# guy3540/Acoustic_Locating_VQ-VAE

Hardware: AMD Instinct MI355X
Metric: spectrograms/sec (train step), speech VQ-VAE default config (higher is better)
Workload: dtype x3mx_hb

## Files before the change

acoustic_locating_vq-vae_amd/csrc/wgrad_reduce.h:

```cpp
#pragma once
#include "alvq_common.h"

namespace alvq {

static __device__ __forceinline__ void wgrad_reduce_body(const float* partial, float* dw, int splits, int KW, int M, int C,
                                                         int w_layout, int accumulate, const float* scale, long stride, int bid,
                                                         int nblk) {
  const long total = (long)KW * M * C;
  const float sc = scale ? *scale : 1.f;
  if (w_layout == ALVQ_W_OIK && KW == 3) {
    const long pairs = (long)M * C;
    for (long q = bid * 256L + threadIdx.x; q < pairs; q += (long)nblk * 256) {
      float s0 = 0.f, s1 = 0.f, s2 = 0.f;
      const float* p = partial + q;
      int k = 0;
      for (; k + 2 <= splits; k += 2) {
        const float* pa = p + (long)k * stride;
        const float* pb = pa + stride;
        const float a0 = pa[0], a1 = pa[pairs], a2 = pa[2 * pairs], b0 = pb[0], b1 = pb[pairs], b2 = pb[2 * pairs];
        s0 = (s0 + a0) + b0;
        s1 = (s1 + a1) + b1;
        s2 = (s2 + a2) + b2;
      }
      for (; k < splits; ++k) {
        const float* pa = p + (long)k * stride;
        s0 += pa[0];
        s1 += pa[pairs];
        s2 += pa[2 * pairs];
      }
      if (scale) { s0 *= sc; s1 *= sc; s2 *= sc; }
      float* o = dw + 3 * q;
      if (accumulate) { s0 += o[0]; s1 += o[1]; s2 += o[2]; }
      o[0] = s0; o[1] = s1; o[2] = s2;
    }
    return;
  }
  for (long e = bid * 256L + threadIdx.x; e < total; e += (long)nblk * 256) {
    int m, c, t;
    if (w_layout == ALVQ_W_OIK) {
      t = (int)(e % KW);
      c = (int)((e / KW) % C);
      m = (int)(e / ((long)KW * C));
    } else {
      const int tt = (int)(e % KW);
      t = KW - 1 - tt;
      m = (int)((e / KW) % M);
      c = (int)(e / ((long)KW * M));
    }
    const long src = ((long)t * M + m) * C + c;
    float s = 0.f;
    int k = 0;
    for (; k + 4 <= splits; k += 4) {
      const float v0 = partial[(long)k * stride + src], v1 = partial[(long)(k + 1) * stride + src],
                  v2 = partial[(long)(k + 2) * stride + src], v3 = partial[(long)(k + 3) * stride + src];
      s = (((s + v0) + v1) + v2) + v3;
    }
    for (; k < splits; ++k) s += partial[(long)k * stride + src];
    if (scale) s *= sc;
    dw[e] = accumulate ? dw[e] + s : s;
  }
}
static __global__ void wgrad_reduce_kernel(const float* partial, float* dw, int splits, int KW, int M, int C, int w_layout,
                                    int accumulate, const float* scale) {
  wgrad_reduce_body(partial, dw, splits, KW, M, C, w_layout, accumulate, scale, (long)KW * M * C, blockIdx.x, gridDim.x);
}

template <int RB>
static __device__ __forceinline__ void wgrad_reduce_iok_body(float (&tile)[3][RB][65], const float* partial, float* dw, int splits,
                                                             int KW, int M, int C, int accumulate, const float* scale, int bid) {
  constexpr int RI = RB / 8;
  const int ctiles = (C + 63) / 64;
  const int m0 = (bid / ctiles) * RB, c0 = (bid % ctiles) * 64;
  const int tx = threadIdx.x & 31, ty = threadIdx.x >> 5;
  const long plane = (long)M * C, total = (long)KW * plane;
  const bool pair = (C % 2 == 0);
  float s0[3][RI], s1[3][RI];
#pragma unroll
  for (int t = 0; t < 3; ++t)
#pragma unroll
    for (int i = 0; i < RI; ++i) s0[t][i] = s1[t][i] = 0.f;
  const int c = c0 + 2 * tx;
  const bool full = pair && m0 + RB <= M && c0 + 64 <= C;
  if (full) {
    const float* p0 = partial + (long)(m0 + ty) * C + c;
    if (KW == 3) {
#pragma unroll 4
      for (int k = 0; k < splits; ++k) {
        float2 v[3][RI];
#pragma unroll
        for (int t = 0; t < 3; ++t)
#pragma unroll
          for (int i = 0; i < RI; ++i) v[t][i] = *(const float2*)(p0 + (long)k * total + (long)t * plane + (long)(8 * i) * C);
#pragma unroll
        for (int t = 0; t < 3; ++t)
#pragma unroll
          for (int i = 0; i < RI; ++i) {
            s0[t][i] += v[t][i].x;
            s1[t][i] += v[t][i].y;
          }
      }
    } else {
#pragma unroll 4
      for (int k = 0; k < splits; ++k) {
        float2 v[RI];
#pragma unroll
        for (int i = 0; i < RI; ++i) v[i] = *(const float2*)(p0 + (long)k * total + (long)(8 * i) * C);
#pragma unroll
        for (int i = 0; i < RI; ++i) {
          s0[0][i] += v[i].x;
          s1[0][i] += v[i].y;
        }
      }
    }
  } else
  for (int k = 0; k < splits; ++k) {
    const float* pk = partial + (long)k * total + c;
#pragma unroll
    for (int t = 0; t < 3; ++t) {
      if (t >= KW) break;
#pragma unroll
      for (int i = 0; i < RI; ++i) {
        const int m = m0 + ty + 8 * i;
        if (m >= M) continue;
        const float* p = pk + (long)t * plane + (long)m * C;
        if (pair && c + 1 < C) {
          const float2 v = *(const float2*)p;
          s0[t][i] += v.x;
          s1[t][i] += v.y;
        } else {
          if (c < C) s0[t][i] += p[0];
          if (c + 1 < C) s1[t][i] += p[1];
        }
      }
    }
  }
#pragma unroll
  for (int t = 0; t < 3; ++t) {
    if (t >= KW) break;
#pragma unroll
    for (int i = 0; i < RI; ++i) {
      tile[t][ty + 8 * i][2 * tx] = s0[t][i];
      tile[t][ty + 8 * i][2 * tx + 1] = s1[t][i];
    }
  }
  __syncthreads();
  const int run = RB * KW;
  for (int e = threadIdx.x; e < 64 * run; e += 256) {
    const int cc = e / run, j = e - cc * run, mr = j / KW, tt = j - mr * KW;
    if (c0 + cc >= C || m0 + mr >= M) continue;
    const long o = ((long)(c0 + cc) * M + m0) * KW + j;
    float v = tile[KW - 1 - tt][mr][cc];
    if (scale) v *= *scale;
    dw[o] = accumulate ? dw[o] + v : v;
  }
}
template <int RB>
static __global__ __launch_bounds__(256) void wgrad_reduce_iok_kernel(const float* partial, float* dw, int splits, int KW,
                                                                      int M, int C, int accumulate, const float* scale) {
  __shared__ float tile[3][RB][65];
  wgrad_reduce_iok_body<RB>(tile, partial, dw, splits, KW, M, C, accumulate, scale, blockIdx.x);
}

static inline void wgrad_reduce_launch(const float* partial, float* dw, int splits, int KW, int M, int C, int w_layout,
                                       int accumulate, hipStream_t s, const float* scale = nullptr) {
  if (w_layout == ALVQ_W_IOK) {
    const int grid = ((M + 15) / 16) * ((C + 63) / 64);
    hipLaunchKernelGGL(wgrad_reduce_iok_kernel<16>, dim3(grid), dim3(256), 0, s, partial, dw, splits, KW, M, C, accumulate, scale);
    return;
  }
  const long total = (long)KW * M * C;
  int rgrid = (int)((total + 255) / 256);
  if (rgrid > 2048) rgrid = 2048;
  hipLaunchKernelGGL(wgrad_reduce_kernel, dim3(rgrid), dim3(256), 0, s, partial, dw, splits, KW, M, C, w_layout, accumulate, scale);
}

}
```

acoustic_locating_vq-vae_amd/csrc/wgrad_reduce_batch.hip:

```cpp
#include "alvq_common.h"
#include "wgrad_reduce.h"

namespace alvq {

constexpr int RB_MAX = 40;
struct ReduceBatch {
  alvq_reduce_desc d[RB_MAX];
  int blk0[RB_MAX];
  int nblk[RB_MAX];
  int n;
};

__global__ __launch_bounds__(256) void wgrad_reduce_batch_kernel(ReduceBatch b) {
  __shared__ float tile[3][16][65];
  int di = 0;
  for (int i = 1; i < b.n; ++i)
    if ((int)blockIdx.x >= b.blk0[i]) di = i;
  const alvq_reduce_desc& d = b.d[di];
  const int lb = blockIdx.x - b.blk0[di];
  const int acc = d.accumulate;
  if (d.w_layout == ALVQ_W_IOK && d.stride == (int64_t)d.KW * d.M * d.C)
    wgrad_reduce_iok_body<16>(tile, d.partial, d.dst, d.splits, d.KW, d.M, d.C, acc, d.scale, lb);
  else
    wgrad_reduce_body(d.partial, d.dst, d.splits, d.KW, d.M, d.C, d.w_layout, acc, d.scale, (long)d.stride, lb, b.nblk[di]);
}

}

using namespace alvq;

extern "C" int alvq_wgrad_reduce_batch(const alvq_reduce_desc* descs, int n, void* stream) {
  ALVQ_REQUIRE(descs && n > 0, ALVQ_EINVAL, "alvq_wgrad_reduce_batch: no descriptors");
  for (int i = 0; i < n; ++i) {
    const alvq_reduce_desc& s = descs[i];
    ALVQ_REQUIRE(s.partial && s.dst, ALVQ_EINVAL, "alvq_wgrad_reduce_batch: null pointer in descriptor %d", i);
    ALVQ_REQUIRE(s.splits >= 1 && s.splits <= 64 && s.M > 0 && s.C > 0 && (s.KW == 1 || s.KW == 3), ALVQ_EINVAL,
                 "alvq_wgrad_reduce_batch: bad dims in descriptor %d", i);
    ALVQ_REQUIRE(s.w_layout == ALVQ_W_OIK || s.w_layout == ALVQ_W_IOK, ALVQ_EINVAL, "alvq_wgrad_reduce_batch: w_layout in descriptor %d", i);
    ALVQ_REQUIRE(s.stride >= (int64_t)s.KW * s.M * s.C, ALVQ_EINVAL, "alvq_wgrad_reduce_batch: stride in descriptor %d", i);
  }
  for (int i0 = 0; i0 < n; i0 += RB_MAX) {
    ReduceBatch b{};
    b.n = n - i0 < RB_MAX ? n - i0 : RB_MAX;
    int blocks = 0;
    for (int i = 0; i < b.n; ++i) {
      const alvq_reduce_desc& s = descs[i0 + i];
      b.d[i] = s;
      const long total = (long)s.KW * s.M * s.C;
      int nb;
      if (s.w_layout == ALVQ_W_IOK && s.stride == total) nb = ((s.M + 15) / 16) * ((s.C + 63) / 64);
      else {
        nb = (int)((total + 255) / 256);
        if (nb > 2048) nb = 2048;
      }
      b.blk0[i] = blocks;
      b.nblk[i] = nb;
      blocks += nb;
    }
    hipLaunchKernelGGL(wgrad_reduce_batch_kernel, dim3(blocks), dim3(256), 0, (hipStream_t)stream, b);
    int rc = check_launch("alvq_wgrad_reduce_batch");
    if (rc) return rc;
  }
  return ALVQ_OK;
}
```

acoustic_locating_vq-vae_amd/src/acoustic_locating_vq_vae/_native.py:

```python
from __future__ import annotations

import collections
import ctypes
import functools
import os

import torch

_LIB = None
_HERE = os.path.dirname(os.path.abspath(__file__))
_DEFAULT_LIB = os.path.normpath(os.path.join(_HERE, "..", "..", "lib", "libalvq.so"))

W_OIK = 0
W_IOK = 1
VQ_PARTIALS = 1024
EW_PARTIALS = 1024

_c_void_p = ctypes.c_void_p
_i32 = ctypes.c_int
_i64 = ctypes.c_int64
_f32 = ctypes.c_float

_SIGNATURES = {
    "alvq_version": (ctypes.c_char_p, []),
# ... 258 lines not shown
        rc = lib().alvq_conv1d_f32(_ptr(x, name="x"), _ptr(w, name="w"), _ptr(bias, name="bias"), _ptr(skip1, name="skip1"),
                                   _ptr(skip2, name="skip2"), _ptr(mask, name="mask"), _ptr(post, name="post"),
                                   _ptr(y), _ptr(y2), B, C, M, L, KW, w_layout, int(bool(relu)), _stream())
    _check(rc, "alvq_conv1d_f32")
    return (y, y2) if post is not None else y


_WS = {}
_WS_RETIRED = []


def _workspace(nbytes, device):
    key = (device.type, device.index, torch.cuda.current_stream(device).cuda_stream)
    buf = _WS.get(key)
    if buf is None or buf.numel() < nbytes:
        if buf is not None:
            _WS_RETIRED.append(buf)
        buf = torch.empty(max(nbytes, 1 << 20), device=device, dtype=torch.uint8)
        _WS[key] = buf
    return buf


WGRAD_DEFER = 2
_ARENA = {}


class ReduceDesc(ctypes.Structure):
    _fields_ = [("partial", ctypes.c_void_p), ("dst", ctypes.c_void_p), ("scale", ctypes.c_void_p), ("splits", ctypes.c_int32),
                ("KW", ctypes.c_int32), ("M", ctypes.c_int32), ("C", ctypes.c_int32), ("w_layout", ctypes.c_int32),
                ("accumulate", ctypes.c_int32), ("stride", ctypes.c_int64)]


def arena_reset(device):
    key = (device.type, device.index, torch.cuda.current_stream(device).cuda_stream)
    st = _ARENA.get(key)
    if st is not None:
        st["chunk"], st["off"] = 0, 0


def arena_alloc(nbytes, device):
    key = (device.type, device.index, torch.cuda.current_stream(device).cuda_stream)
    st = _ARENA.setdefault(key, {"chunks": [], "chunk": 0, "off": 0})
    nbytes = (nbytes + 255) // 256 * 256
    while True:
        if st["chunk"] >= len(st["chunks"]):
            st["chunks"].append(torch.empty(max(nbytes, 256 << 20), device=device, dtype=torch.uint8))
            st["off"] = 0
        buf = st["chunks"][st["chunk"]]
        if st["off"] + nbytes <= buf.numel():
            ptr = buf.data_ptr() + st["off"]
            st["off"] += nbytes
            return ptr
        st["chunk"] += 1
        st["off"] = 0


class DeferredReductions(list):

    def __init__(self):
        super().__init__()
        self.keep = []


def wgrad_reduce_batch(descs):
    if not descs:
        return
    arr = (ReduceDesc * len(descs))(*descs)
    _check(lib().alvq_wgrad_reduce_batch(ctypes.addressof(arr), len(descs), _stream()), "alvq_wgrad_reduce_batch")
    if isinstance(descs, DeferredReductions):
        descs.keep.clear()


def _defer_descs(defer, ws_ptr, dw, dbias, scale, nseg, B, C, M, L, KW, w_layout):
    L_ = lib()
    scale_ptr = _sptr(scale, 1)
    dsts = {dw.data_ptr()} | ({dbias.data_ptr()} if dbias is not None else set())
    if any(d.dst in dsts for d in defer):
        wgrad_reduce_batch(defer)
        del defer[:]
    if scale is not None and hasattr(defer, "keep"):
        defer.keep.append(scale)
    splits = L_.alvq_conv1d_wgrad_bf16_splits(B, C, M, L, KW, nseg, int(dbias is not None))
    defer.append(ReduceDesc(ws_ptr, dw.data_ptr(), scale_ptr, splits, KW, M, C, w_layout, 1, KW * M * C))
    if dbias is not None:
        off = L_.alvq_conv1d_wgrad_bf16_bias_offset(B, C, M, L, KW)
        defer.append(ReduceDesc(ws_ptr + off, dbias.data_ptr(), scale_ptr, splits, 1, 1, M, W_OIK, 1, (M + 63) // 64 * 64))


def conv1d_wgrad(dy, x, KW, w_layout=W_OIK, want_bias=False, dw_out=None, dbias_out=None, accumulate=False):
# ... 1054 lines not shown
```

acoustic_locating_vq-vae_amd/src/acoustic_locating_vq_vae/_ops.py:

```python
from __future__ import annotations

import os

import numpy as np
import torch

from . import _native as N

OIK, IOK = N.W_OIK, N.W_IOK

DEFAULT_DTYPE = "x3mx_hb"
MODES = ("x3mx_hb", "f16mx_hb", "bf16x3_hb", "f32", "bf16")
INTERNAL_MODES = ("f16mx", "bf16x3", "f16mx_hd")
_DTYPE = os.environ.get("ALVQ_DTYPE", DEFAULT_DTYPE)
if _DTYPE not in MODES:
    raise ValueError("ALVQ_DTYPE must be one of %s, got %r" % (", ".join(repr(m) for m in MODES), _DTYPE))


def set_compute_dtype(name, internal=False):
    global _DTYPE
    if name not in MODES and not (internal and name in INTERNAL_MODES):
        raise ValueError("compute dtype must be one of %s, got %r" % (", ".join(repr(m) for m in MODES), name))
    _DTYPE = name

# ... 15 lines not shown
    for p in params:
        if p.grad is not None:
            _GRAD_SINKS[p.data_ptr()] = p.grad


_SINKS_ACTIVE = 0


class use_grad_sinks:

    def __enter__(self):
        global _SINKS_ACTIVE
        _SINKS_ACTIVE += 1

    def __exit__(self, *exc):
        global _SINKS_ACTIVE
        _SINKS_ACTIVE -= 1


_DEFERRED = None


class deferred_reduce:
    def __enter__(self):
        global _DEFERRED
        self.prev, _DEFERRED = _DEFERRED, (N.DeferredReductions() if os.environ.get("ALVQ_DEFER_REDUCE", "1") != "0" else None)
        return _DEFERRED

    def __exit__(self, *exc):
        global _DEFERRED
        _DEFERRED = self.prev


_API_FORWARDS = 0


def note_training_forward(device):
    global _API_FORWARDS
    if device.type != "cuda" or _SINKS_ACTIVE or not has_fp16_range() or torch.cuda.is_current_stream_capturing():
        return
    every = int(os.environ.get("ALVQ_RANGE_CHECK_EVERY", "200"))
    _API_FORWARDS += 1
    if every <= 0 or _API_FORWARDS < every:
        return
    _API_FORWARDS = 0
    flag = N.f16mx_range_flag(reset=True, device=device)
    if flag:
        import warnings
        warnings.warn("acoustic_locating_vq_vae: fp16 range flag %d in mode %s -- a value entering or produced inside the "
# ... 136 lines not shown
    def __exit__(self, *exc):
        global _LATENT_TAP
        _LATENT_TAP = self.prev



class use_pack_pool:

    def __init__(self, pool, refresh=True):
        self.pool, self.do_refresh = pool, refresh

    def __enter__(self):
        global _ACTIVE_POOL
        self.prev, _ACTIVE_POOL = _ACTIVE_POOL, self.pool
        if self.pool is not None and self.do_refresh:
            self.pool.refresh()

    def __exit__(self, *exc):
        global _ACTIVE_POOL
        _ACTIVE_POOL = self.prev


def _defer_kw(eng, sink):
    return {"defer": _DEFERRED} if (_DEFERRED is not None and sink is not None and eng.can_defer) else {}


def _wgrad(eng, dy, x, kw, layout, w, b=None, dw_prev=None):
    if b is not None and not b.requires_grad:
        b = None
    if not w.requires_grad:
        if b is None:
            return None, None
        raise RuntimeError("a convolution with a frozen weight and a trainable bias is not supported on the HIP path")
    sw, sb = _sink(w), _sink(b)
    if sw is not None and (b is None or sb is not None):
        eng.wgrad(dy, x, kw, layout, want_bias=b is not None, dw_out=sw, dbias_out=sb, accumulate=True, **_defer_kw(eng, sw))
        return None, None
    if b is not None:
        dw, db = eng.wgrad(dy, x, kw, layout, want_bias=True, dw_out=dw_prev, accumulate=dw_prev is not None)
        return dw, db
    return eng.wgrad(dy, x, kw, layout, dw_out=dw_prev, accumulate=dw_prev is not None), None


def dense(x):
    if isinstance(x, StandardisedT):
        return x.materialise()
    if x.dtype != torch.float32:
# ... 560 lines not shown
```

acoustic_locating_vq-vae_amd/src/acoustic_locating_vq_vae/train_step.py:

```python
from __future__ import annotations

import os

import torch
import torch.distributed as dist

from . import _native as N
from . import _ops

_ALIGN = 64


def _round_up(n):
    return (n + _ALIGN - 1) // _ALIGN * _ALIGN


def _world_rank(group=None, without=(1, 0)):
    if not (dist.is_available() and dist.is_initialized()):
        return without
    return dist.get_world_size(group), dist.get_rank(group)


def unique_trainable(params):
    seen, out = set(), []
# ... 9 lines not shown
    def __init__(self, params, extra=0):
        self.params = unique_trainable(params)
        if not self.params:
            raise ValueError("no trainable parameters")
        dev = self.params[0].device
        self.offsets, total = [], _ALIGN
        for p in self.params:
            if p.device != dev or p.dtype != torch.float32:
                raise ValueError("all parameters must be fp32 on one device")
            self.offsets.append(total)
            total += _round_up(p.numel())
        self.extra_span = (total, total + extra) if extra else None
        total += _round_up(extra)
        self.numel = sum(p.numel() for p in self.params)
        self.flat = torch.zeros(total, device=dev, dtype=torch.float32)
        self.grad = torch.zeros(total, device=dev, dtype=torch.float32)
        for p, off in zip(self.params, self.offsets):
            n = p.numel()
            self.flat[off:off + n].copy_(p.data.reshape(-1))
            p.data = self.flat[off:off + n].view(p.shape)
            p.grad = self.grad[off:off + n].view(p.shape)
        self.skip_slot = self.grad[0:1]

    def zero_grad(self):
        if self.grad.is_cuda:
            N.fill_(self.grad, 0.0)
        else:
            self.grad.zero_()
        for p, off in zip(self.params, self.offsets):
            if p.grad is None or p.grad.data_ptr() != self.grad.data_ptr() + 4 * off:
                p.grad = self.grad[off:off + p.numel()].view(p.shape)

    def sync_grads(self, group=None, force=False):
        world = _world_rank(group, without=(0, 0))[0]
        if world == 0 or (world == 1 and not force):
            return 1.0
        dist.all_reduce(self.grad, op=dist.ReduceOp.SUM, group=group)
        return 1.0 / world

    def span(self, params):
        ids = {id(p) for p in params}
        idx = [i for i, p in enumerate(self.params) if id(p) in ids]
        if not idx or idx != list(range(idx[0], idx[-1] + 1)) or len(idx) != len(ids):
            raise ValueError("bucket parameters are not a contiguous run of the flat buffer")
        last = idx[-1]
        hi = self.offsets[last + 1] if last + 1 < len(self.offsets) else self.grad.numel()
        return (0 if idx[0] == 0 else self.offsets[idx[0]]), hi

    def sync_span(self, lo, hi, group=None, force=False):
        world = _world_rank(group, without=(0, 0))[0]
        if world == 0 or (world == 1 and not force):
            return None
        return dist.all_reduce(self.grad[lo:hi], op=dist.ReduceOp.SUM, group=group, async_op=True)

    def broadcast_params(self, src=0, group=None):
        if _world_rank(group)[0] > 1:
            dist.broadcast(self.flat, src=src, group=group)


class WarmupCosine:

    __slots__ = ("warmup_steps", "total_steps", "lr_min")

    def __init__(self, warmup_steps, total_steps=None, lr_min=0.0):
        if int(warmup_steps) != warmup_steps or warmup_steps < 0:
            raise ValueError("WarmupCosine: warmup_steps=%r must be an integer >= 0" % (warmup_steps,))
        if total_steps is not None and (int(total_steps) != total_steps or total_steps <= warmup_steps):
            raise ValueError("WarmupCosine: total_steps=%r must be an integer beyond warmup_steps=%r" % (total_steps, warmup_steps))
        if not lr_min >= 0:
            raise ValueError("WarmupCosine: lr_min=%r must be >= 0" % (lr_min,))
        self.warmup_steps = int(warmup_steps)
        self.total_steps = None if total_steps is None else int(total_steps)
        self.lr_min = float(lr_min)

    def __repr__(self):
        return "WarmupCosine(warmup_steps=%d, total_steps=%r, lr_min=%g)" % (self.warmup_steps, self.total_steps, self.lr_min)


def _check_step_controls(max_grad_norm, schedule):
    if max_grad_norm is not None and not float(max_grad_norm) > 0:
# ... 131 lines not shown
        self.opt.prepare(self.grad_scale)
        self.buffers.zero_grad()
        with _ops.use_grad_sinks():
            location = self.model(codes)
            loss = F.mse_loss(location, torch.as_tensor(theta).float().to(location.device) / torch.pi, reduction="mean")
            loss.backward()
        self.buffers.sync_grads(self.group)
        self.opt.clip(_ALIGN, self.buffers.grad.numel())
        self.opt.apply()
        return loss.detach()


def shard_batch(x, rank, world):
    b = x.shape[0]
    if b % world != 0:
        raise ValueError("global batch %d is not divisible by world size %d" % (b, world))
    per = b // world
    return x[rank * per:(rank + 1) * per]


class Trainer:

    def __init__(self, model, kind="speech", lr=1e-3, group=None, grad_buckets=None, force_collective=None,
                 range_check_every=None, strict_range=None, max_grad_norm=None, lr_schedule=None):
        _check_step_controls(max_grad_norm, lr_schedule)
        self.model, self.kind, self.group = model, kind, group
        self.range_check_every = int(os.environ.get("ALVQ_RANGE_CHECK_EVERY", "200")) if range_check_every is None \
            else int(range_check_every)
        self.strict_range = (os.environ.get("ALVQ_RANGE_STRICT", "0") != "0") if strict_range is None else bool(strict_range)
        self.skipped_steps = 0
        self._steps_since_check = 0
        self.force_collective = (os.environ.get("ALVQ_FORCE_COLLECTIVE", "0") != "0") if force_collective is None \
            else bool(force_collective)
        self._echoed_train_encoder = bool(getattr(model, "flag_train_encoder", False)) if kind == "echoed" else None
        params = model._decoder.parameters() if (kind == "echoed" and not self._echoed_train_encoder) else model.parameters()
        from .vq_vae.vector_quantizer import VectorQuantizerEMA
        self._ema = [m for m in model.modules() if isinstance(m, VectorQuantizerEMA)] if kind != "echoed" else []
        self._restart = [m for m in self._ema if m.restarts_enabled()]
        self.buffers = FlatBuffers(params, extra=sum(_ops.EMASink.span_len(m) for m in self._ema))
        self._trainable = [p.requires_grad for p in self.buffers.params]
        world, rank = _world_rank(group)
        self._ema_sinks, off = {}, self.buffers.extra_span[0] if self._ema else 0
        for m in self._ema:
            self._ema_sinks[id(m)] = _ops.EMASink(m, self.buffers.grad, off, rank, world)
            off += _ops.EMASink.span_len(m)
        if world > 1:
            for m in self._restart:
                m._restart_gen.manual_seed(m._restart_seed + rank)
        if self.buffers.flat.is_cuda:
            _ops.register_grad_sinks(self.buffers.params)
        use_pool = self.buffers.flat.is_cuda and os.environ.get("ALVQ_PACK_POOL", "1") != "0"
        self.pack_pool = _ops.PackPool(list(model.parameters()), dynamic=self.buffers.params) if use_pool else None
        self.buffers.broadcast_params(group=group)
        self._broadcast_ema()
        self.opt = FlatAdam(self.buffers, lr=lr, guard=os.environ.get("ALVQ_SKIP_SATURATED", "1") != "0",
                            max_grad_norm=max_grad_norm, schedule=lr_schedule)
        self.grad_scale = 1.0 / world
        self._one = None
        self._buckets = self._cut = self._graph = None
        want_buckets = int(os.environ.get("ALVQ_GRAD_BUCKETS", "1")) if grad_buckets is None else grad_buckets
        if want_buckets >= 2 and kind != "echoed" and hasattr(model, "_encoder") and hasattr(model, "_pre_vq_conv"):
            late = unique_trainable(list(model._encoder.parameters()) + list(model._pre_vq_conv.parameters()))
            late_ids = {id(p) for p in late}
            early = [p for p in self.buffers.params if id(p) not in late_ids]
            if late and early:
                self._late_params, self._early_params = late, early
                self._buckets = (self.buffers.span(early), self.buffers.span(late))
                xs = self.buffers.extra_span
                if xs is not None and not any(lo <= xs[0] and xs[1] <= hi for lo, hi in self._buckets):
                    raise RuntimeError("the EMA statistics span (restart candidates included) is not inside one gradient bucket")

    def preprocess(self, raw, wiener=None):
        if self.kind == "speech":
            x = N.standardise(_ops.dense(raw), take_abs=True)
            return x, x
        if self.kind == "rir":
            x = _ops.StandardisedT(_ops.dense(raw))
            w = wiener.float()
            tgt = N.standardise(w.unsqueeze(2).contiguous()).view(w.shape[0], 1, w.shape[1])
            return x, tgt
        x = N.standardise(_ops.dense(raw))
# ... 9 lines not shown
        return recon_error + vq_loss, recon_error, perplexity

    def _check_frozen(self):
        if [p.requires_grad for p in self.buffers.params] != self._trainable:
            raise RuntimeError("requires_grad of a parameter changed after the Trainer was built; build a new Trainer")
        if self.kind == "echoed" and bool(self.model.flag_train_encoder) != self._echoed_train_encoder:
            raise RuntimeError("set_train_encoder(%s) was called after the Trainer was built; build a new Trainer so "
                               "the encoders' parameters are (not) part of the optimiser" % self.model.flag_train_encoder)

    def _adam_skip(self):
        skip = [self.buffers.extra_span] if self.buffers.extra_span is not None else []
        ids = {id(p): i for i, p in enumerate(self.buffers.params)}
        for m in self.model.modules():
            if hasattr(m, "_train_vq") and not m._train_vq and id(m._embedding.weight) in ids:
                i = ids[id(m._embedding.weight)]
                skip.append((self.buffers.offsets[i], self.buffers.offsets[i] + m._embedding.weight.numel()))
        return skip

    def _body(self, raw, wiener):
        if self.buffers.flat.is_cuda:
            N.arena_reset(self.buffers.flat.device)
        for sink in self._ema_sinks.values():
            sink.written = False
        with _ops.use_pack_pool(self.pack_pool), _ops.use_grad_sinks(), _ops.deferred_reduce() as reductions, \
                _ops.use_ema_sinks(self._ema_sinks):
            x, target = self.preprocess(raw, wiener)
            self.buffers.zero_grad()
            if self._one is None or self._one.device != x.device:
                self._one = torch.ones((), device=x.device)
            if self._buckets is None:
                loss, recon_error, perplexity = self.forward_loss(x, target)
                loss.backward(self._one)
            else:
                with _ops.latent_tap() as tap:
                    loss, recon_error, perplexity = self.forward_loss(x, target)
                loss.backward(self._one)
                self._cut = tap[0] if tap else None
            if reductions:
                N.wgrad_reduce_batch(reductions)
            if self._cut is None:
                self._post_verdict()
        return loss.detach(), recon_error.detach(), perplexity.detach()

    def _post_verdict(self):
        if self.opt.guard and _ops.has_fp16_range():
            N.range_flag_to_slot(self.buffers.skip_slot)

    def _body_late(self):
        if self._cut is None:
            return
        z, leaf = self._cut
        self._cut = None
        with _ops.use_pack_pool(self.pack_pool, refresh=False), _ops.use_grad_sinks(), _ops.deferred_reduce() as reductions:
            z.backward(leaf.grad)
            if reductions:
                N.wgrad_reduce_batch(reductions)
            self._post_verdict()

    def _sync_early(self):
        return self.buffers.sync_span(*self._buckets[0], group=self.group, force=self.force_collective) if self._buckets else None

    def _finish(self, early_work=None):
        if self._buckets is None:
            self.buffers.sync_grads(self.group, force=self.force_collective)
        else:
            late_work = self.buffers.sync_span(*self._buckets[1], group=self.group, force=self.force_collective)
            for w in (early_work, late_work):
                if w is not None:
                    w.wait()
        if self.opt.max_grad_norm is not None:
            xs = self.buffers.extra_span
            self.opt.clip(_ALIGN, xs[0] if xs is not None else self.buffers.grad.numel())
        if self.pack_pool is not None:
            self.opt.apply(self._adam_skip(), pack_pool=self.pack_pool)
        else:
            self.opt.apply(self._adam_skip())
        for m in self._ema:
            sink = self._ema_sinks[id(m)]
            if sink.written:
# ... 80 lines not shown
                for j in self._graph_jitters:
                    j.refresh()
            return self._eager_step(raw, wiener)
        self._static_raw.copy_(raw, non_blocking=True)
        if wiener is not None:
            self._static_wiener.copy_(wiener, non_blocking=True)
        for j in self._graph_jitters:
            j.refresh()
        for m, (rows, n) in zip(self._restart, self._graph_restart):
            m.draw_restart_rows(rows, n)
        self.opt.prepare(self.grad_scale)
        self._graph.replay()
        early = self._sync_early()
        if self._graph_late is not None:
            self._graph_late.replay()
        self._finish(early)
        return self._static_out

    def _eager_step(self, raw, wiener):
        self.opt.prepare(self.grad_scale)
        out = self._body(raw, wiener)
        early = self._sync_early()
        self._body_late()
        self._finish(early)
        return out

    def init_codebook(self, raw_batches, wiener_batches=None, **kmeans_kwargs):
        if self.kind == "echoed":
            raise NotImplementedError("init_codebook: the echoed model's frozen sub-codebooks are out of scope")
        single = isinstance(raw_batches, torch.Tensor)
        raws = [raw_batches] if single else list(raw_batches)
        if wiener_batches is None:
            wieners = [None] * len(raws)
        else:
            wieners = [wiener_batches] if isinstance(wiener_batches, torch.Tensor) else list(wiener_batches)
        if self.kind == "rir" and (len(wieners) != len(raws) or any(w is None for w in wieners)):
            raise ValueError("init_codebook: kind='rir' needs one Wiener batch per raw batch")
        world, rank = _world_rank(self.group)
        weight = self.model._vq._embedding.weight
        km = None
        if rank == 0:
            km = self.model.init_codebook([self.preprocess(r, w)[0] for r, w in zip(raws, wieners)], **kmeans_kwargs)
        if world > 1:
            dist.broadcast(weight.data, src=dist.get_global_rank(self.group, 0) if self.group is not None else 0,
                           group=self.group)
            if self._ema:
# ... 51 lines not shown
```

include/alvq.h:

```cpp
#ifndef ALVQ_H
#define ALVQ_H

#include <stdint.h>

#ifdef __cplusplus
extern "C" {
#endif

#define ALVQ_OK 0
#define ALVQ_EINVAL (-1)
#define ALVQ_EUNSUPPORTED (-2)

#define ALVQ_W_OIK 0
#define ALVQ_W_IOK 1

#define ALVQ_F32 0
#define ALVQ_BF16 1

const char* alvq_version(void);
const char* alvq_last_error(void);

int alvq_set_option(const char* name, int64_t value);
int64_t alvq_get_option(const char* name);

// ... 196 lines not shown
int alvq_rows_to_nlc(const float* x, void* y, int B, int C, int L, int fmt, int standardise, int take_abs, void* stream);
int alvq_rows_to_nlc_max_std_rows(void);

int alvq_ncl_to_nlc_bf16(const float* x, void* y, int B, int C, int L, void* stream);

int alvq_nlc_to_ncl_f32(const void* x, float* y, int B, int C, int L, void* stream);

int alvq_relu_mask_bf16(const void* dy, const void* t, void* out, int64_t n, void* stream);

int alvq_conv1d_bf16(const void* x, const void* wp, const float* bias, const void* skip1, const void* skip2,
                     const void* mask, const void* post, void* y, void* y2, float* y_ncl,
                     int B, int C, int M, int L, int KW, int relu, const void* mask_bits, void* relu_bits_out,
                     void* stream);

int64_t alvq_conv1d_wgrad_bf16_workspace_bytes(int B, int C, int M, int L, int KW);
int alvq_conv1d_wgrad_bf16(const void* dy, const void* x, float* dw, float* dbias, void* workspace,
                           int B, int C, int M, int L, int KW, int w_layout, int accumulate, void* stream);

int alvq_conv1d_wgrad_bf16_multi(const void* const* dy, const void* const* x, int nseg, float* dw, void* workspace,
                                 int B, int C, int M, int L, int KW, int w_layout, int accumulate, void* stream);
int alvq_conv1d_wgrad_bf16_splits(int B, int C, int M, int L, int KW, int nseg, int with_bias);

#define ALVQ_WGRAD_DEFER 2
int64_t alvq_conv1d_wgrad_bf16_bias_offset(int B, int C, int M, int L, int KW);
typedef struct alvq_reduce_desc {
  const float* partial;
  float* dst;
  const float* scale;
  int32_t splits, KW, M, C, w_layout, accumulate;
  int64_t stride;
} alvq_reduce_desc;
int alvq_wgrad_reduce_batch(const alvq_reduce_desc* descs, int n, void* stream);

int64_t alvq_nlc_plane_bytes(int B, int L, int C);
int alvq_pack_weight_bf16x3(const float* w, void* wp, int M, int C, int KW, int w_layout, void* stream);
int alvq_ncl_to_nlc_bf16x3(const float* x, void* y, int B, int C, int L, void* stream);
int alvq_nlc_to_ncl_bf16x3(const void* x, float* y, int B, int C, int L, void* stream);
int alvq_relu_mask_bf16x3(const void* dy, const void* t, void* out, int B, int C, int L, void* stream);
int alvq_conv1d_bf16x3(const void* x, const void* wp, const float* bias, const void* skip1, const void* skip2,
                       const void* mask, const void* post, void* y, void* y2, float* y_ncl,
                       int B, int C, int M, int L, int KW, int relu, void* stream);
int64_t alvq_conv1d_wgrad_bf16x3_workspace_bytes(int B, int C, int M, int L, int KW);
int alvq_conv1d_wgrad_bf16x3(const void* dy, const void* x, float* dw, float* dbias, void* workspace,
                             int B, int C, int M, int L, int KW, int w_layout, int accumulate, void* stream);
int alvq_conv1d_wgrad_bf16x3_multi(const void* const* dy, const void* const* x, int nseg, float* dw, void* workspace,
                                   int B, int C, int M, int L, int KW, int w_layout, int accumulate, void* stream);
// ... 45 lines not shown
```

Measured before the change: 7941.

## Skip full gradient zeroing by storing first deferred reductions and zeroing only gaps

The trainer learns from the first step which flat-gradient spans are written by deferred weight-grad reductions. On later steps it zeroes only the uncovered gaps, using a new zero-descriptor kind in the batched reduce kernel, and marks the first reduction into each span as a plain store instead of read-modify-write. The tiled reduce kernel is also generalised to the OIK layout, with float4 loads and stores, so the batched reduce takes a vectorised tile path for most layers. The cost is extra planning logic with fallback re-zeroing when the reduction pattern changes. Stale gradients are possible if the plan is wrong.

```diff
diff --git a/acoustic_locating_vq-vae_amd/csrc/wgrad_reduce.h b/acoustic_locating_vq-vae_amd/csrc/wgrad_reduce.h
--- a/acoustic_locating_vq-vae_amd/csrc/wgrad_reduce.h
+++ b/acoustic_locating_vq-vae_amd/csrc/wgrad_reduce.h
@@ -2,6 +2,12 @@
 #include "alvq_common.h"
 
 namespace alvq {
+
+constexpr int WR_STORE = 0, WR_ACCUMULATE = 1, WR_STORE_ZEROED = 2;
+static __device__ __forceinline__ float wgrad_reduce_out(float v, const float* o, int accumulate) {
+  if (accumulate == WR_STORE) return v;
+  return (accumulate == WR_STORE_ZEROED ? 0.f : *o) + v;
+}
 
 static __device__ __forceinline__ void wgrad_reduce_body(const float* partial, float* dw, int splits, int KW, int M, int C,
                                                          int w_layout, int accumulate, const float* scale, long stride, int bid,
@@ -30,8 +36,9 @@
       }
       if (scale) { s0 *= sc; s1 *= sc; s2 *= sc; }
       float* o = dw + 3 * q;
-      if (accumulate) { s0 += o[0]; s1 += o[1]; s2 += o[2]; }
-      o[0] = s0; o[1] = s1; o[2] = s2;
+      o[0] = wgrad_reduce_out(s0, o, accumulate);
+      o[1] = wgrad_reduce_out(s1, o + 1, accumulate);
+      o[2] = wgrad_reduce_out(s2, o + 2, accumulate);
     }
     return;
   }
@@ -57,7 +64,7 @@
     }
     for (; k < splits; ++k) s += partial[(long)k * stride + src];
     if (scale) s *= sc;
-    dw[e] = accumulate ? dw[e] + s : s;
+    dw[e] = wgrad_reduce_out(s, dw + e, accumulate);
   }
 }
 static __global__ void wgrad_reduce_kernel(const float* partial, float* dw, int splits, int KW, int M, int C, int w_layout,
@@ -65,110 +72,191 @@
   wgrad_reduce_body(partial, dw, splits, KW, M, C, w_layout, accumulate, scale, (long)KW * M * C, blockIdx.x, gridDim.x);
 }
 
-template <int RB>
-static __device__ __forceinline__ void wgrad_reduce_iok_body(float (&tile)[3][RB][65], const float* partial, float* dw, int splits,
-                                                             int KW, int M, int C, int accumulate, const float* scale, int bid) {
-  constexpr int RI = RB / 8;
-  const int ctiles = (C + 63) / 64;
-  const int m0 = (bid / ctiles) * RB, c0 = (bid % ctiles) * 64;
-  const int tx = threadIdx.x & 31, ty = threadIdx.x >> 5;
+constexpr int WR_ROWS = 16, WR_COLS = 64;
+typedef float WgradReduceTile[3][WR_ROWS][WR_COLS + 1];
+
+static __host__ __device__ __forceinline__ bool wgrad_reduce_tiled(int w_layout, int KW, int M, int C, long stride) {
+  if (stride != (long)KW * M * C) return false;
+  return w_layout == ALVQ_W_IOK || (C % 4 == 0 && M >= WR_ROWS && C >= WR_COLS);
+}
+static __host__ __device__ __forceinline__ int wgrad_reduce_tiles(int M, int C) {
+  return ((M + WR_ROWS - 1) / WR_ROWS) * ((C + WR_COLS - 1) / WR_COLS);
+}
+
+template <int KW, int NS>
+static __device__ __forceinline__ void wgrad_reduce_quads(const float* p0, int splits, long total, long plane, f32x4 (&s)[3]) {
+  int k = 0;
+  for (; k + NS <= splits; k += NS) {
+    f32x4 v[NS][KW];
+#pragma unroll
+    for (int u = 0; u < NS; ++u)
+#pragma unroll
+      for (int t = 0; t < KW; ++t) v[u][t] = *(const f32x4*)(p0 + (long)(k + u) * total + (long)t * plane);
+#pragma unroll
+    for (int u = 0; u < NS; ++u)
+#pragma unroll
+      for (int t = 0; t < KW; ++t) s[t] += v[u][t];
+  }
+  for (; k < splits; ++k) {
+    f32x4 v[KW];
+#pragma unroll
+    for (int t = 0; t < KW; ++t) v[t] = *(const f32x4*)(p0 + (long)k * total + (long)t * plane);
+#pragma unroll
+    for (int t = 0; t < KW; ++t) s[t] += v[t];
+  }
+}
+
+static __device__ __forceinline__ void wgrad_reduce_tile_body(WgradReduceTile& tile, const float* partial, float* dw, int splits,
+                                                              int KW, int M, int C, int w_layout, int accumulate,
+                                                              const float* scale, int bid) {
+  constexpr int RI = WR_ROWS / 8;
+  const int ctiles = (C + WR_COLS - 1) / WR_COLS;
+  const int m0 = (bid / ctiles) * WR_ROWS, c0 = (bid % ctiles) * WR_COLS;
   const long plane = (long)M * C, total = (long)KW * plane;
-  const bool pair = (C % 2 == 0);
-  float s0[3][RI], s1[3][RI];
-#pragma unroll
-  for (int t = 0; t < 3; ++t)
-#pragma unroll
-    for (int i = 0; i < RI; ++i) s0[t][i] = s1[t][i] = 0.f;
-  const int c = c0 + 2 * tx;
-  const bool full = pair && m0 + RB <= M && c0 + 64 <= C;
-  if (full) {
-    const float* p0 = partial + (long)(m0 + ty) * C + c;
-    if (KW == 3) {
-#pragma unroll 4
-      for (int k = 0; k < splits; ++k) {
-        float2 v[3][RI];
-#pragma unroll
-        for (int t = 0; t < 3; ++t)
-#pragma unroll
-          for (int i = 0; i < RI; ++i) v[t][i] = *(const float2*)(p0 + (long)k * total + (long)t * plane + (long)(8 * i) * C);
-#pragma unroll
-        for (int t = 0; t < 3; ++t)
-#pragma unroll
-          for (int i = 0; i < RI; ++i) {
-            s0[t][i] += v[t][i].x;
-            s1[t][i] += v[t][i].y;
-          }
-      }
-    } else {
-#pragma unroll 4
-      for (int k = 0; k < splits; ++k) {
-        float2 v[RI];
-#pragma unroll
-        for (int i = 0; i < RI; ++i) v[i] = *(const float2*)(p0 + (long)k * total + (long)(8 * i) * C);
-#pragma unroll
-        for (int i = 0; i < RI; ++i) {
-          s0[0][i] += v[i].x;
-          s1[0][i] += v[i].y;
-        }
-      }
-    }
-  } else
-  for (int k = 0; k < splits; ++k) {
-    const float* pk = partial + (long)k * total + c;
+  const bool whole = m0 + WR_ROWS <= M && c0 + WR_COLS <= C;
+  const bool quad = whole && C % 4 == 0 && ((uintptr_t)partial & 15) == 0;
+  if (quad) {
+    const int tx = threadIdx.x & 15, ty = threadIdx.x >> 4;
+    f32x4 s[3];
+#pragma unroll
+    for (int t = 0; t < 3; ++t) s[t] = f32x4{0.f, 0.f, 0.f, 0.f};
+    const float* p0 = partial + (long)(m0 + ty) * C + c0 + 4 * tx;
+    if (KW == 3) wgrad_reduce_quads<3, 4>(p0, splits, total, plane, s);
+    else wgrad_reduce_quads<1, 8>(p0, splits, total, plane, s);
 #pragma unroll
     for (int t = 0; t < 3; ++t) {
       if (t >= KW) break;
 #pragma unroll
+      for (int q = 0; q < 4; ++q) tile[t][ty][4 * tx + q] = s[t][q];
+    }
+  } else {
+    const int tx = threadIdx.x & 31, ty = threadIdx.x >> 5;
+    const bool pair = C % 2 == 0 && ((uintptr_t)partial & 7) == 0;
+    float s0[3][RI], s1[3][RI];
+#pragma unroll
+    for (int t = 0; t < 3; ++t)
+#pragma unroll
+      for (int i = 0; i < RI; ++i) s0[t][i] = s1[t][i] = 0.f;
+    const int c = c0 + 2 * tx;
+    if (pair && whole) {
+      const float* p0 = partial + (long)(m0 + ty) * C + c;
+      if (KW == 3) {
+#pragma unroll 4
+        for (int k = 0; k < splits; ++k) {
+          float2 v[3][RI];
+#pragma unroll
+          for (int t = 0; t < 3; ++t)
+#pragma unroll
+            for (int i = 0; i < RI; ++i) v[t][i] = *(const float2*)(p0 + (long)k * total + (long)t * plane + (long)(8 * i) * C);
+#pragma unroll
+          for (int t = 0; t < 3; ++t)
+#pragma unroll
+            for (int i = 0; i < RI; ++i) {
+              s0[t][i] += v[t][i].x;
+              s1[t][i] += v[t][i].y;
+            }
+        }
+      } else {
+#pragma unroll 4
+        for (int k = 0; k < splits; ++k) {
+          float2 v[RI];
+#pragma unroll
+          for (int i = 0; i < RI; ++i) v[i] = *(const float2*)(p0 + (long)k * total + (long)(8 * i) * C);
+#pragma unroll
+          for (int i = 0; i < RI; ++i) {
+            s0[0][i] += v[i].x;
+            s1[0][i] += v[i].y;
+          }
+        }
+      }
+    } else
+    for (int k = 0; k < splits; ++k) {
+      const float* pk = partial + (long)k * total + c;
+#pragma unroll
+      for (int t = 0; t < 3; ++t) {
+        if (t >= KW) break;
+#pragma unroll
+        for (int i = 0; i < RI; ++i) {
+          const int m = m0 + ty + 8 * i;
+          if (m >= M) continue;
+          const float* p = pk + (long)t * plane + (long)m * C;
+          if (pair && c + 1 < C) {
+            const float2 v = *(const float2*)p;
+            s0[t][i] += v.x;
+            s1[t][i] += v.y;
+          } else {
+            if (c < C) s0[t][i] += p[0];
+            if (c + 1 < C) s1[t][i] += p[1];
+          }
+        }
+      }
+    }
+#pragma unroll
+    for (int t = 0; t < 3; ++t) {
+      if (t >= KW) break;
+#pragma unroll
       for (int i = 0; i < RI; ++i) {
-        const int m = m0 + ty + 8 * i;
-        if (m >= M) continue;
-        const float* p = pk + (long)t * plane + (long)m * C;
-        if (pair && c + 1 < C) {
-          const float2 v = *(const float2*)p;
-          s0[t][i] += v.x;
-          s1[t][i] += v.y;
-        } else {
-          if (c < C) s0[t][i] += p[0];
-          if (c + 1 < C) s1[t][i] += p[1];
-        }
-      }
-    }
-  }
-#pragma unroll
-  for (int t = 0; t < 3; ++t) {
-    if (t >= KW) break;
-#pragma unroll
-    for (int i = 0; i < RI; ++i) {
-      tile[t][ty + 8 * i][2 * tx] = s0[t][i];
-      tile[t][ty + 8 * i][2 * tx + 1] = s1[t][i];
+        tile[t][ty + 8 * i][2 * tx] = s0[t][i];
+        tile[t][ty + 8 * i][2 * tx + 1] = s1[t][i];
+      }
     }
   }
   __syncthreads();
-  const int run = RB * KW;
-  for (int e = threadIdx.x; e < 64 * run; e += 256) {
+  const float sc = scale ? *scale : 1.f;
+  if (w_layout == ALVQ_W_OIK) {
+    const int run = WR_COLS * KW;
+    if (quad && ((uintptr_t)dw & 15) == 0) {
+      for (int e = 4 * threadIdx.x; e < WR_ROWS * run; e += 4 * 256) {
+        const int mr = e / run, j = e - mr * run;
+        float* o = dw + ((long)(m0 + mr) * C + c0) * KW + j;
+        f32x4 v, old = {0.f, 0.f, 0.f, 0.f};
+        if (accumulate == WR_ACCUMULATE) old = *(const f32x4*)o;
+#pragma unroll
+        for (int q = 0; q < 4; ++q) {
+          const int cc = (j + q) / KW, t = (j + q) - cc * KW;
+          float x = tile[t][mr][cc];
+          if (scale) x *= sc;
+          v[q] = accumulate == WR_STORE ? x : old[q] + x;
+        }
+        *(f32x4*)o = v;
+      }
+      return;
+    }
+    for (int e = threadIdx.x; e < WR_ROWS * run; e += 256) {
+      const int mr = e / run, j = e - mr * run, cc = j / KW, t = j - cc * KW;
+      if (c0 + cc >= C || m0 + mr >= M) continue;
+      const long o = ((long)(m0 + mr) * C + c0) * KW + j;
+      float v = tile[t][mr][cc];
+      if (scale) v *= sc;
+      dw[o] = wgrad_reduce_out(v, dw + o, accumulate);
+    }
+    return;
+  }
+  const int run = WR_ROWS * KW;
+  for (int e = threadIdx.x; e < WR_COLS * run; e += 256) {
     const int cc = e / run, j = e - cc * run, mr = j / KW, tt = j - mr * KW;
     if (c0 + cc >= C || m0 + mr >= M) continue;
     const long o = ((long)(c0 + cc) * M + m0) * KW + j;
     float v = tile[KW - 1 - tt][mr][cc];
-    if (scale) v *= *scale;
-    dw[o] = accumulate ? dw[o] + v : v;
-  }
-}
-template <int RB>
-static __global__ __launch_bounds__(256) void wgrad_reduce_iok_kernel(const float* partial, float* dw, int splits, int KW,
-                                                                      int M, int C, int accumulate, const float* scale) {
-  __shared__ float tile[3][RB][65];
-  wgrad_reduce_iok_body<RB>(tile, partial, dw, splits, KW, M, C, accumulate, scale, blockIdx.x);
+    if (scale) v *= sc;
+    dw[o] = wgrad_reduce_out(v, dw + o, accumulate);
+  }
+}
+static __global__ __launch_bounds__(256) void wgrad_reduce_tile_kernel(const float* partial, float* dw, int splits, int KW, int M,
+                                                                       int C, int w_layout, int accumulate, const float* scale) {
+  __shared__ WgradReduceTile tile;
+  wgrad_reduce_tile_body(tile, partial, dw, splits, KW, M, C, w_layout, accumulate, scale, blockIdx.x);
 }
 
 static inline void wgrad_reduce_launch(const float* partial, float* dw, int splits, int KW, int M, int C, int w_layout,
                                        int accumulate, hipStream_t s, const float* scale = nullptr) {
-  if (w_layout == ALVQ_W_IOK) {
-    const int grid = ((M + 15) / 16) * ((C + 63) / 64);
-    hipLaunchKernelGGL(wgrad_reduce_iok_kernel<16>, dim3(grid), dim3(256), 0, s, partial, dw, splits, KW, M, C, accumulate, scale);
+  accumulate = accumulate ? WR_ACCUMULATE : WR_STORE;
+  const long total = (long)KW * M * C;
+  if (wgrad_reduce_tiled(w_layout, KW, M, C, total)) {
+    hipLaunchKernelGGL(wgrad_reduce_tile_kernel, dim3(wgrad_reduce_tiles(M, C)), dim3(256), 0, s, partial, dw, splits, KW, M, C,
+                       w_layout, accumulate, scale);
     return;
   }
-  const long total = (long)KW * M * C;
   int rgrid = (int)((total + 255) / 256);
   if (rgrid > 2048) rgrid = 2048;
   hipLaunchKernelGGL(wgrad_reduce_kernel, dim3(rgrid), dim3(256), 0, s, partial, dw, splits, KW, M, C, w_layout, accumulate, scale);
diff --git a/acoustic_locating_vq-vae_amd/csrc/wgrad_reduce_batch.hip b/acoustic_locating_vq-vae_amd/csrc/wgrad_reduce_batch.hip
--- a/acoustic_locating_vq-vae_amd/csrc/wgrad_reduce_batch.hip
+++ b/acoustic_locating_vq-vae_amd/csrc/wgrad_reduce_batch.hip
@@ -12,15 +12,18 @@
 };
 
 __global__ __launch_bounds__(256) void wgrad_reduce_batch_kernel(ReduceBatch b) {
-  __shared__ float tile[3][16][65];
+  __shared__ WgradReduceTile tile;
   int di = 0;
   for (int i = 1; i < b.n; ++i)
     if ((int)blockIdx.x >= b.blk0[i]) di = i;
   const alvq_reduce_desc& d = b.d[di];
   const int lb = blockIdx.x - b.blk0[di];
-  const int acc = d.accumulate;
-  if (d.w_layout == ALVQ_W_IOK && d.stride == (int64_t)d.KW * d.M * d.C)
-    wgrad_reduce_iok_body<16>(tile, d.partial, d.dst, d.splits, d.KW, d.M, d.C, acc, d.scale, lb);
+  const int acc = d.accumulate == WR_STORE_ZEROED || d.accumulate == WR_STORE ? d.accumulate : WR_ACCUMULATE;
+  if (d.splits == 0) {
+    const long total = (long)d.KW * d.M * d.C;
+    for (long e = lb * 256L + threadIdx.x; e < total; e += b.nblk[di] * 256L) d.dst[e] = 0.f;
+  } else if (wgrad_reduce_tiled(d.w_layout, d.KW, d.M, d.C, (long)d.stride))
+    wgrad_reduce_tile_body(tile, d.partial, d.dst, d.splits, d.KW, d.M, d.C, d.w_layout, acc, d.scale, lb);
   else
     wgrad_reduce_body(d.partial, d.dst, d.splits, d.KW, d.M, d.C, d.w_layout, acc, d.scale, (long)d.stride, lb, b.nblk[di]);
 }
@@ -33,9 +36,11 @@
   ALVQ_REQUIRE(descs && n > 0, ALVQ_EINVAL, "alvq_wgrad_reduce_batch: no descriptors");
   for (int i = 0; i < n; ++i) {
     const alvq_reduce_desc& s = descs[i];
-    ALVQ_REQUIRE(s.partial && s.dst, ALVQ_EINVAL, "alvq_wgrad_reduce_batch: null pointer in descriptor %d", i);
-    ALVQ_REQUIRE(s.splits >= 1 && s.splits <= 64 && s.M > 0 && s.C > 0 && (s.KW == 1 || s.KW == 3), ALVQ_EINVAL,
+    ALVQ_REQUIRE(s.dst && (s.partial || s.splits == 0), ALVQ_EINVAL, "alvq_wgrad_reduce_batch: null pointer in descriptor %d", i);
+    ALVQ_REQUIRE(s.splits >= 0 && s.splits <= 64 && s.M > 0 && s.C > 0 && (s.KW == 1 || s.KW == 3), ALVQ_EINVAL,
                  "alvq_wgrad_reduce_batch: bad dims in descriptor %d", i);
+    ALVQ_REQUIRE(s.splits > 0 || (!s.partial && !s.scale && s.accumulate == 0), ALVQ_EINVAL,
+                 "alvq_wgrad_reduce_batch: descriptor %d has no splits: the zero kind takes no partials, no scale and accumulate = 0", i);
     ALVQ_REQUIRE(s.w_layout == ALVQ_W_OIK || s.w_layout == ALVQ_W_IOK, ALVQ_EINVAL, "alvq_wgrad_reduce_batch: w_layout in descriptor %d", i);
     ALVQ_REQUIRE(s.stride >= (int64_t)s.KW * s.M * s.C, ALVQ_EINVAL, "alvq_wgrad_reduce_batch: stride in descriptor %d", i);
   }
@@ -48,7 +53,7 @@
       b.d[i] = s;
       const long total = (long)s.KW * s.M * s.C;
       int nb;
-      if (s.w_layout == ALVQ_W_IOK && s.stride == total) nb = ((s.M + 15) / 16) * ((s.C + 63) / 64);
+      if (s.splits > 0 && wgrad_reduce_tiled(s.w_layout, s.KW, s.M, s.C, (long)s.stride)) nb = wgrad_reduce_tiles(s.M, s.C);
       else {
         nb = (int)((total + 255) / 256);
         if (nb > 2048) nb = 2048;
diff --git a/acoustic_locating_vq-vae_amd/src/acoustic_locating_vq_vae/_native.py b/acoustic_locating_vq-vae_amd/src/acoustic_locating_vq_vae/_native.py
--- a/acoustic_locating_vq-vae_amd/src/acoustic_locating_vq_vae/_native.py
+++ b/acoustic_locating_vq-vae_amd/src/acoustic_locating_vq_vae/_native.py
@@ -304,6 +304,7 @@
 
 
 WGRAD_DEFER = 2
+REDUCE_STORE_ZEROED = 2
 _ARENA = {}
 
 
@@ -339,14 +340,29 @@
 
 class DeferredReductions(list):
 
-    def __init__(self):
+    def __init__(self, store_first=None):
         super().__init__()
         self.keep = []
+        self.store_first = set(store_first) if store_first else None
+        self.log = []
+
+    def claim(self):
+        for d in self:
+            if self.store_first and d.dst in self.store_first:
+                self.store_first.discard(d.dst)
+                d.accumulate = REDUCE_STORE_ZEROED
+            self.log.append((d.dst, d.KW * d.M * d.C))
+
+
+def reduce_zero_desc(dst_ptr, nfloats):
+    return ReduceDesc(None, dst_ptr, None, 0, 1, 1, nfloats, W_OIK, 0, nfloats)
 
 
 def wgrad_reduce_batch(descs):
     if not descs:
         return
+    if isinstance(descs, DeferredReductions):
+        descs.claim()
     arr = (ReduceDesc * len(descs))(*descs)
     _check(lib().alvq_wgrad_reduce_batch(ctypes.addressof(arr), len(descs), _stream()), "alvq_wgrad_reduce_batch")
     if isinstance(descs, DeferredReductions):
diff --git a/acoustic_locating_vq-vae_amd/src/acoustic_locating_vq_vae/_ops.py b/acoustic_locating_vq-vae_amd/src/acoustic_locating_vq_vae/_ops.py
--- a/acoustic_locating_vq-vae_amd/src/acoustic_locating_vq_vae/_ops.py
+++ b/acoustic_locating_vq-vae_amd/src/acoustic_locating_vq_vae/_ops.py
@@ -61,9 +61,14 @@
 
 
 class deferred_reduce:
+
+    def __init__(self, store_first=None):
+        self.store_first = store_first
+
     def __enter__(self):
         global _DEFERRED
-        self.prev, _DEFERRED = _DEFERRED, (N.DeferredReductions() if os.environ.get("ALVQ_DEFER_REDUCE", "1") != "0" else None)
+        self.prev, _DEFERRED = _DEFERRED, (N.DeferredReductions(self.store_first)
+                                           if os.environ.get("ALVQ_DEFER_REDUCE", "1") != "0" else None)
         return _DEFERRED
 
     def __exit__(self, *exc):
@@ -246,7 +251,14 @@
 
 
 def _defer_kw(eng, sink):
-    return {"defer": _DEFERRED} if (_DEFERRED is not None and sink is not None and eng.can_defer) else {}
+    if _DEFERRED is None or sink is None:
+        return {}
+    if eng.can_defer:
+        return {"defer": _DEFERRED}
+    if _DEFERRED.store_first and sink.data_ptr() in _DEFERRED.store_first:
+        raise RuntimeError("a weight-gradient launch that cannot defer its reduction accumulates into a gradient the step's "
+                           "plan stores into (train_step.UpdateTailPlan); build the Trainer with store_grads=False")
+    return {}
 
 
 def _wgrad(eng, dy, x, kw, layout, w, b=None, dw_prev=None):
diff --git a/acoustic_locating_vq-vae_amd/src/acoustic_locating_vq_vae/train_step.py b/acoustic_locating_vq-vae_amd/src/acoustic_locating_vq_vae/train_step.py
--- a/acoustic_locating_vq-vae_amd/src/acoustic_locating_vq_vae/train_step.py
+++ b/acoustic_locating_vq-vae_amd/src/acoustic_locating_vq_vae/train_step.py
@@ -55,8 +55,14 @@
             p.grad = self.grad[off:off + n].view(p.shape)
         self.skip_slot = self.grad[0:1]
 
-    def zero_grad(self):
-        if self.grad.is_cuda:
+    def zero_spans(self, spans):
+        base = self.grad.data_ptr()
+        N.wgrad_reduce_batch([N.reduce_zero_desc(base + 4 * lo, hi - lo) for lo, hi in spans if hi > lo])
+
+    def zero_grad(self, spans=None):
+        if self.grad.is_cuda and spans is not None:
+            self.zero_spans(spans)
+        elif self.grad.is_cuda:
             N.fill_(self.grad, 0.0)
         else:
             self.grad.zero_()
@@ -89,6 +95,50 @@
     def broadcast_params(self, src=0, group=None):
         if _world_rank(group)[0] > 1:
             dist.broadcast(self.flat, src=src, group=group)
+
+
+class UpdateTailPlan:
+
+    __slots__ = ("lists", "stores", "zeros", "key")
+
+    def __init__(self, lists, stores, zeros, key):
+        self.lists, self.stores, self.zeros, self.key = lists, stores, zeros, key
+
+    def matches(self, part, reductions):
+        return tuple(reductions) == self.lists[part]
+
+    def zeros_of(self, bucket):
+        return tuple((lo, hi) for lo, hi in self.zeros if bucket[0] <= lo and hi <= bucket[1])
+
+
+def plan_update_tail(total, reductions, param_spans, buckets=None, key=None):
+    params = {off: n for off, n in param_spans}
+    lists = tuple(tuple((int(off), int(n)) for off, n in part) for part in reductions)
+    seen, stores = {}, []
+    for p, part in enumerate(lists):
+        mine = []
+        for off, n in part:
+            if off in seen:
+                continue
+            if params.get(off) != n or off < 0 or off + n > total:
+                return None
+            if buckets is not None and not (p < len(buckets) and buckets[p][0] <= off and off + n <= buckets[p][1]):
+                return None
+            seen[off] = n
+            mine.append((off, n))
+        stores.append(tuple(mine))
+    if not seen:
+        return None
+    cuts = sorted({0, total} | ({e for b in buckets for e in b} if buckets is not None else set()))
+    zeros, lo = [], 0
+    for off in sorted(seen) + [total]:
+        if off < lo:
+            return None
+        for a, b in zip(cuts, cuts[1:]):
+            if max(lo, a) < min(off, b):
+                zeros.append((max(lo, a), min(off, b)))
+        lo = off + seen.get(off, 0)
+    return UpdateTailPlan(lists, tuple(stores), tuple(zeros), key)
 
 
 class WarmupCosine:
@@ -266,7 +316,7 @@
 class Trainer:
 
     def __init__(self, model, kind="speech", lr=1e-3, group=None, grad_buckets=None, force_collective=None,
-                 range_check_every=None, strict_range=None, max_grad_norm=None, lr_schedule=None):
+                 range_check_every=None, strict_range=None, max_grad_norm=None, lr_schedule=None, store_grads=None):
         _check_step_controls(max_grad_norm, lr_schedule)
         self.model, self.kind, self.group = model, kind, group
         self.range_check_every = int(os.environ.get("ALVQ_RANGE_CHECK_EVERY", "200")) if range_check_every is None \
@@ -301,6 +351,10 @@
                             max_grad_norm=max_grad_norm, schedule=lr_schedule)
         self.grad_scale = 1.0 / world
         self._one = None
+        self.store_grads = (os.environ.get("ALVQ_STORE_GRADS", "1") != "0") if store_grads is None else bool(store_grads)
+        self._tail_plan = None
+        self._tail_live = None
+        self._tail_logs = [None, None]
         self._buckets = self._cut = self._graph = None
         want_buckets = int(os.environ.get("ALVQ_GRAD_BUCKETS", "1")) if grad_buckets is None else grad_buckets
         if want_buckets >= 2 and kind != "echoed" and hasattr(model, "_encoder") and hasattr(model, "_pre_vq_conv"):
@@ -356,10 +410,12 @@
             N.arena_reset(self.buffers.flat.device)
         for sink in self._ema_sinks.values():
             sink.written = False
-        with _ops.use_pack_pool(self.pack_pool), _ops.use_grad_sinks(), _ops.deferred_reduce() as reductions, \
+        plan = self._tail_live = self._tail_usable()
+        self._tail_logs = [None, None]
+        with _ops.use_pack_pool(self.pack_pool), _ops.use_grad_sinks(), _ops.deferred_reduce(self._tail_first(0)) as reductions, \
                 _ops.use_ema_sinks(self._ema_sinks):
             x, target = self.preprocess(raw, wiener)
-            self.buffers.zero_grad()
+            self.buffers.zero_grad(plan.zeros if plan is not None else None)
             if self._one is None or self._one.device != x.device:
                 self._one = torch.ones((), device=x.device)
             if self._buckets is None:
@@ -370,11 +426,50 @@
                     loss, recon_error, perplexity = self.forward_loss(x, target)
                 loss.backward(self._one)
                 self._cut = tap[0] if tap else None
-            if reductions:
-                N.wgrad_reduce_batch(reductions)
+            self._reduce_part(reductions, 0)
             if self._cut is None:
+                self._reduce_part(None, 1)
                 self._post_verdict()
         return loss.detach(), recon_error.detach(), perplexity.detach()
+
+    def _tail_key(self):
+        if not (self.store_grads and self.buffers.grad.is_cuda) or os.environ.get("ALVQ_DEFER_REDUCE", "1") == "0":
+            return None
+        return (_ops.get_compute_dtype(),)
+
+    def _tail_usable(self):
+        if self._tail_plan is not None and self._tail_plan.key != self._tail_key():
+            self._tail_plan = None
+        return self._tail_plan
+
+    def _tail_done(self):
+        return {off for log in self._tail_logs if log for off, _ in log}
+
+    def _tail_first(self, part):
+        plan = self._tail_live
+        if plan is None:
+            return None
+        done, base = self._tail_done(), self.buffers.grad.data_ptr()
+        return {base + 4 * off for stores in plan.stores[part:] for off, _ in stores if off not in done}
+
+    def _reduce_part(self, reductions, part):
+        plan, base = self._tail_live, self.buffers.grad.data_ptr()
+        if reductions:
+            N.wgrad_reduce_batch(reductions)
+        log = None if reductions is None else [((dst - base) // 4, n) for dst, n in reductions.log]
+        self._tail_logs[part] = log
+        if plan is not None and not plan.matches(part, log or ()):
+            done = self._tail_done()
+            self.buffers.zero_spans([(off, off + n) for off, n in plan.stores[part] if off not in done])
+            self._tail_plan = None
+
+    def _tail_learn(self):
+        key = self._tail_key()
+        if self._tail_plan is not None or key is None or self._tail_logs[0] is None:
+            return
+        b = self.buffers
+        self._tail_plan = plan_update_tail(b.grad.numel(), [self._tail_logs[0], self._tail_logs[1] or []],
+                                           [(off, p.numel()) for p, off in zip(b.params, b.offsets)], self._buckets, key)
 
     def _post_verdict(self):
         if self.opt.guard and _ops.has_fp16_range():
@@ -385,10 +480,10 @@
             return
         z, leaf = self._cut
         self._cut = None
-        with _ops.use_pack_pool(self.pack_pool, refresh=False), _ops.use_grad_sinks(), _ops.deferred_reduce() as reductions:
+        with _ops.use_pack_pool(self.pack_pool, refresh=False), _ops.use_grad_sinks(), \
+                _ops.deferred_reduce(self._tail_first(1)) as reductions:
             z.backward(leaf.grad)
-            if reductions:
-                N.wgrad_reduce_batch(reductions)
+            self._reduce_part(reductions, 1)
             self._post_verdict()
 
     def _sync_early(self):
@@ -515,6 +610,7 @@
         out = self._body(raw, wiener)
         early = self._sync_early()
         self._body_late()
+        self._tail_learn()
         self._finish(early)
         return out
 
diff --git a/include/alvq.h b/include/alvq.h
--- a/include/alvq.h
+++ b/include/alvq.h
@@ -242,6 +242,7 @@
 int alvq_conv1d_wgrad_bf16_splits(int B, int C, int M, int L, int KW, int nseg, int with_bias);
 
 #define ALVQ_WGRAD_DEFER 2
+#define ALVQ_REDUCE_STORE_ZEROED 2
 int64_t alvq_conv1d_wgrad_bf16_bias_offset(int B, int C, int M, int L, int KW);
 typedef struct alvq_reduce_desc {
   const float* partial;
```

Result: no change. 7968, median of 6 (+0.3%).
